# fukangl/SMG-multimodal-grasping

Hardware: AMD Instinct MI355X
Metric: affordance fwd+bwd passes/sec (16-rot 224^2 RGB-D) (higher is better)
Workload: dtype f32; 1 GPU; 16 rot x 224^2 (S=640): fwd + Huber + bwd + Adam per GPU per step; reinforcement_net style 0; 17 trunk passes; fp32; leg=headline, rotations=16, input_size=640, parallelism=dp1

## Files before the change

### smg-multimodal-grasping_amd/csrc/backward.hip

```cpp
#include "engine.h"

int do_backward(smg_engine* e, const smg_net* net, const float* dq, hipStream_t st, int phases, bool elem_head) {
    if (!e->have_fwd) return fail(-22, "smg_backward without a preceding smg_forward");
    if (!net->grads) return fail(-22, "net.grads is NULL");
    if (phases == 2 && !e->bw_phase0_done)
        return fail(-22, "smg_backward_phase(1) must follow smg_backward_phase(0) of the same forward");
    if ((phases & 1) && e->bw_phase0_done)
        return fail(-22, "smg_backward / smg_backward_phase(0) while the second half of a two-phase backward is still due (run phase 1 or a new forward)");
    const Layout& L = *e->L;
    const TrunkRef& T = L.trunk[e->f_trunk];
    const HeadRef& Hd = L.head[e->f_head];
    const int NS = e->f_streams, NP = e->f_pairs;
    const float* P = net->params;
    float* Gr = net->grads;
    const Plane p4 = e->p_blk[3];
    const bool ph_a = phases & 1, ph_b = phases & 2;
    if (ph_a) {
        for (int r = 0; r < kStatRep; ++r) HIP_OK(hipMemsetAsync(e->bstat + (size_t)r * kStatRepStride, 0, 2 * e->bstat_span * sizeof(double), st));
    }
    const bool split16 = e->prec == 0 && kSplitOp == 3;
    if (ph_a && split16) HIP_OK(hipMemsetAsync(e->gamax, 0, (size_t)e->gamax_words * sizeof(unsigned), st));
    const hipStream_t s2 = (e->prof || e->serialize) ? st : e->side;
    auto fork = [&](hipEvent_t ev) -> int {
        HIP_OK(hipEventRecord(ev, st));
// ... 96 lines not shown
        return LayerBuf{e->GS[r % kRing], e->D2[r % kRing], e->D2S[r % kRing], r};
    };
    auto fused_gsrc = [&](int b, const DenseLayerRef& d) {
        const int Ct = kBlockCtot[b];
        GradSrc g{};
        g.g = el(e, e->G[b], d.cin); g.ldg = Ct; g.x = el(e, e->X[b], d.cin); g.ldx = Ct;
        g.xsum = fsum(e, e->st_X[b]) + d.cin; g.xsq = fsq(e, e->st_X[b]) + d.cin;
        g.s1 = b1(e, e->st_X[b]) + d.cin; g.s2 = b2(e, e->st_X[b]) + d.cin; g.sstride = Ct; g.eps = kEps;
        return g;
    };
    auto issue_wgrads = [&](int b, int i) -> int {
        const Plane pl = e->p_blk[b];
        const int Ct = kBlockCtot[b];
        const DenseLayerRef& d = T.layers[b][i];
        float* bt = el(e, e->Bt, e->bt_off[b][i]);
        const LayerBuf lb = buf_of(b, i);
        const WgradPlan w = plan_layer_wgrads(pl, d.cin, NS, e->prec, split16, e->deterministic, e->part_floats, e->generic3x3, e->generic_w1);
        GradSrc gsrc{};
        if (gs_on_side(pl)) launch_gs_apply(b, i, s2, lb.GS);
        if (gs_materialised) { gsrc.g = lb.GS; gsrc.ldg = kGrowth; gsrc.amax = gamax_of(e, b, i, 0); }
        else gsrc = fused_gsrc(b, d);
        if (!e->generic3x3) {
            const PartialTiles::Slot at = tiles.place_halo3x3(w.w3.groups);
            if (at.refused) return fail(-12, tiles.refusal());
            launch_reduce2(e, s2, at.first);
            Halo3x3WgradArgs a;
            a.g = gsrc; a.pl = pl; a.src = bt; a.C = kBottleneck;
            a.bt = bn_table(e, e->sb_tab[b][i], e->max_streams, 0, kBottleneck, P + d.n2.w, P + d.n2.b);
            a.asc = asc_n2(e, b, i);
            a.tiles_x = w.w3.tiles_x; a.n_tiles = w.w3.n_tiles; a.tiles_per_wg = w.w3.tiles_per_wg;
            a.part = part_at(e, at);
            a.groups = w.w3.groups; a.streams = NS;
            const double flops = 2.0 * NS * pl.HW * 9 * kBottleneck * kGrowth, bytes = ESZ(e) * NS * pl.HW * (kGrowth + kBottleneck);
            if (w.w3.ts == 16) {
                PREC_DISPATCH(e, launch_kernel(e, conv3x3_halo_wgrad_kernel<16, PREC>, dim3(w.w3_grid), dim3(256), HaloWgradSGeo<16, PREC>::smem_bytes(), s2,
                                               K_W3, flops, bytes, false, a));
            } else {
                PREC_DISPATCH(e, launch_kernel(e, conv3x3_halo_wgrad_kernel<8, PREC>, dim3(w.w3_grid), dim3(256), HaloWgradSGeo<8, PREC>::smem_bytes(), s2,
                                               K_W3, flops, bytes, false, a));
            }
            launch_reduce2(e, s2, tiles.launched(at, reduce_tap_inner(a.part, w.w3.groups * NS, Gr + d.c2.w)));
        } else {
            int chunk, cps;
            pick_chunk(pl, NS, 9, chunk, cps);
            BwdWeightP<CfgW32x128, W_THREE, C_3x3, kPdWgrad, false> p{};
            p.gbuf = lb.GS; p.ldg = kGrowth; p.gcoff = 0; p.xbuf = nullptr; p.pa = pl; p.MA = kGrowth;
            p.bbuf = bt; p.ldb = kBottleneck; p.pb = pl; p.NB = kBottleneck;
            p.bsum = fsum(e, e->st_Bt[b][i]); p.bsq = fsq(e, e->st_Bt[b][i]); p.bstride = kBottleneck;
            p.bgamma = P + d.n2.w; p.bbeta = P + d.n2.b; p.eps = kEps;
            p.chunk = chunk; p.chunks_per_stream = cps; p.n_chunks = NS * cps;
            p.dw = Gr + d.c2.w; p.ldw_out = kBottleneck * 9;
            const dim3 grid(1, 1, 9 * NS * cps);
            if (int rc = launch_wgrad(e, s2, p, grid, K_W3, 2.0 * NS * pl.HW * 9 * kBottleneck * kGrowth,
                                      ESZ(e) * NS * pl.HW * (kGrowth + kBottleneck), 9, C_3x3, tiles, tiles.place_alone(wgrad_partial_floats(p, grid)))) return rc;
        }
        if (w.w1_ws) {
            using G = WswGeo;
            static_assert(G::BN == kW1WsTileN, "plan_layer_wgrads counts this kernel's column tiles");
            Wgrad1x1WsArgs a{};
            a.d2 = reinterpret_cast<const u32x4*>(lb.D2); a.binv = lb.D2S; a.x = e->X[b]; a.ldb = Ct; a.pl = pl; a.NB = d.cin;
            a.btab = stat_table(e, e->sx_tab[b], e->max_streams, Ct); a.bgamma = P + d.n1.w; a.bbeta = P + d.n1.b; a.basc = asc_n1(e, b, i);
            a.chunk = w.chunk; a.chunks_per_stream = w.cps; a.n_chunks = NS * w.cps;
            a.dw = Gr + d.c1.w; a.ldw_out = d.cin; a.ldp = w.nt * G::BN;
            const PartialTiles::Slot at = tiles.place_behind3x3((int64_t)a.n_chunks * G::BM * a.ldp);
            launch_reduce2(e, s2, at.first);
            if (at.refused) return fail(-12, tiles.refusal());
            a.part = part_at(e, at);
            a.tm = TileMap{a.n_chunks, w.nt, 0};
            launch_kernel(e, conv1x1_wgrad_ws_kernel, dim3(tile_grid(a.tm)), dim3(512), G::smem_bytes(w.chunk), s2, K_W1,
                          2.0 * NS * pl.HW * d.cin * kBottleneck, 4.0 * NS * pl.HW * (kBottleneck + d.cin), false, a);
            ReduceArgs red1{};
            if (a.part) red1 = reduce_chunk_major(a.part, a.n_chunks, 1, G::BM, d.cin, G::BM, a.ldp, a.dw, d.cin, C_IDENT);
            launch_reduce2(e, s2, tiles.launched(at, red1));
        } else {
            using Cfg = CfgW128x64;
            static_assert(Cfg::BN == kW1TileN, "plan_layer_wgrads counts this kernel's column tiles");
            auto go = [&](auto ptag) -> int {
                BwdWeightP<MC<Cfg, decltype(ptag)::value>, W_ONE, C_IDENT, kPdWgrad, false, decltype(ptag)::value> p{};
                p.gbuf = lb.D2; p.ldg = kBottleneck; p.gcoff = 0; p.xbuf = nullptr; p.pa = pl; p.MA = kBottleneck; p.binv = lb.D2S; p.basc = asc_n1(e, b, i);
                p.bbuf = e->X[b]; p.ldb = Ct; p.pb = pl; p.NB = d.cin;
                p.bsum = fsum(e, e->st_X[b]); p.bsq = fsq(e, e->st_X[b]); p.bstride = Ct; p.btab = stat_table(e, e->sx_tab[b], e->max_streams, Ct);
                p.bgamma = P + d.n1.w; p.bbeta = P + d.n1.b; p.eps = kEps;
                p.chunk = w.chunk; p.chunks_per_stream = w.cps; p.n_chunks = NS * w.cps;
                p.dw = Gr + d.c1.w; p.ldw_out = d.cin;
                const dim3 grid(1, w.nt, NS * w.cps);
                return launch_wgrad(e, s2, p, grid, K_W1, 2.0 * NS * pl.HW * d.cin * kBottleneck,
                                    ESZ(e) * NS * pl.HW * (kBottleneck + d.cin), 1, C_IDENT, tiles, tiles.place_behind3x3(wgrad_partial_floats(p, grid)));
            };
            PREC_DISPATCH(e, if (int rc = go(PTAG)) return rc);
        }
        return 0;
    };
    auto debug_stop = [&]() -> int {
        launch_reduce2(e, s2, tiles.drain());
        HIP_OK(hipEventRecord(e->ev_end, s2));
        HIP_OK(hipStreamWaitEvent(st, e->ev_end, 0));
        if (int rc = walk_status(e)) return rc;
        e->have_fwd = false; e->bw_phase0_done = false; e->prof_stage = -1;
        return 0;
    };
    const bool pooled_tail = e->prec == 0 && e->f_stem1 && !e->stem_plane_tail && (NS > 4 || e->deterministic);
    for (int b = ph_a ? 3 : 0; b >= (ph_b ? 0 : 1); --b) {
        e->prof_stage = b;
        const Plane pl = e->p_blk[b];
        const int Ct = kBlockCtot[b];
        if (e->dbg_stop == b * 100 + 50) return debug_stop();
        if (b == 0 && pooled_tail) {
            StemMomArgs a;
            a.img = e->img4; a.pi = e->p_img; a.ps = e->p_stem; a.part = e->mom_part;
            a.tiles_x = stem_mom_tiles_x(e->p_stem); a.n_tiles = stem_mom_tiles(e->p_stem); a.tiles_per_wg = kMomTilesPerWg;
            if (fork(e->ev_misc)) return -5;
            e->prof_stage = -1;
            launch_kernel(e, stem_moments_kernel, dim3(e->mom_groups, NS), dim3(256), 0, s2, K_OTHER, 0, 0, false, a);
            launch_kernel(e, stem_moments_sum_kernel, dim3((kMomOut + 255) / 256, NS), dim3(256), 0, s2, K_OTHER, 0, 0, false,
                          (const float*)e->mom_part, e->mom_groups, e->mom);
            e->prof_stage = b;
        }
        for (int i = (int)T.layers[b].size() - 1; i >= 0; --i) {
            const DenseLayerRef& d = T.layers[b][i];
            float* bt = el(e, e->Bt, e->bt_off[b][i]);
// ... 262 lines not shown
```

### smg-multimodal-grasping_amd/csrc/engine.h

```cpp
#pragma once
#include <hip/hip_runtime.h>

#include <algorithm>
#include <cmath>
#include <cstdio>
#include <cstdlib>
#include <cstring>
#include <string>
#include <type_traits>
#include <vector>

#include "../../include/smg_hip.h"
#include "elem.cuh"
#include "scene.cuh"
#include "gemm.cuh"
#include "halo.cuh"
#include "ws.cuh"
#include "wsw.cuh"
#include "plan.h"

using namespace smg;

int smg_fail(int code, const std::string& msg);
static inline int fail(int code, const std::string& msg) { return smg_fail(code, msg); }
// ... 23 lines not shown
using CfgW64x64 = GemmCfg<64, 64, 16, 2, 2, 1, false>;
using CfgW64x256 = GemmCfg<64, 256, 16, 2, 2, 1, false>;

template <class C, int PREC, int MUL = 2>
using MC = typename std::conditional<PREC == 0, C, GemmCfg<C::BM, C::BN, MUL * C::BK, C::WM, C::WN, C::WK, C::AT>>::type;
enum Kind {
    K_STEM = 0, K_C1, K_C3, K_TRANS, K_HEAD0, K_D3, K_W3, K_D1, K_W1, K_TW, K_TD, K_SW, K_HW0, K_HD0, K_OTHER, K_COUNT
};
static const char* kKindNames[K_COUNT] = {"stem7x7_fwd", "conv1x1_fwd", "conv3x3_fwd", "transition_fwd", "head_conv0_fwd",
                                          "conv3x3_dgrad", "conv3x3_wgrad", "conv1x1_dgrad", "conv1x1_wgrad",
                                          "transition_wgrad", "transition_dgrad", "stem_wgrad", "head_conv0_wgrad",
                                          "head_conv0_dgrad", "elementwise"};

constexpr int kGroup = GROUP_MAX;
constexpr int kRing = kGroup + 2;

constexpr int kDbRep = 8;
struct DbSeg { int64_t grad_off; int scr_off; int n; };

struct ProfRec { hipEvent_t a, b; int kind; double flops; int stage; double bytes; };

struct StatArr { int64_t off; int stride; };

struct smg_engine {
    int device = 0, S = 0, max_streams = 0, max_pairs = 0, head_out = 1;
    Plane p_img, p_stem, p_blk[4];
    int OH = 1, OW = 1;
    const Layout* L = nullptr;

    float* img4 = nullptr; float* stem = nullptr; float* X[4] = {}; float* Bt = nullptr;
    std::vector<int64_t> bt_off[4];
    unsigned char* argmax = nullptr;
    float* F = nullptr; float* H1 = nullptr;
    float* G[4] = {}; float* GS[kRing] = {}; float* D2[kRing] = {}; float* part = nullptr; int64_t part_floats = 0;
    float* DY2 = nullptr; float* D2S[kRing] = {};
    hipStream_t side = nullptr; hipEvent_t ev_gs[kRing] = {}, ev_d2[kRing] = {}, ev_side[kRing] = {}, ev_misc = nullptr, ev_end = nullptr; float* DY0 = nullptr; float* DH1 = nullptr; float* DF = nullptr;
    double* fstat = nullptr; int64_t fstat_span = 0;
    double* bstat = nullptr; int64_t bstat_span = 0;
    float* dbscr = nullptr; int db_total = 0; int db_off[4][24] = {}; int db_toff[3] = {}; struct DbSeg* d_dbseg = nullptr; int n_dbseg = 0;
    StatArr st_stem, st_X[4], st_F, st_H1; std::vector<StatArr> st_Bt[4];
    u32x4* packed_u = nullptr; int64_t packed_units = 0;
    float* packed_f = nullptr; int64_t packed_floats = 0;
    PackDesc* d_pack = nullptr; std::vector<PackDesc> h_pack[3]; std::vector<PackDesc> h_pack_head[3];
    int pack_stride = 0, bnupd_stride = 0, n_bnupd = 0;
    int64_t pk_conv0 = 0, pk_conv0_1 = 0, pk_head0 = 0, pk_hd0 = 0, pk_head1 = 0;
    std::vector<int64_t> pk_c1[4], pk_d1[4], pk_g3f[4], pk_g3d[4], pk_hf[4], pk_hd[4]; int64_t pk_t[3] = {}, pk_td[3] = {};
    int max_pack = 0;
    float* asc = nullptr; ActScaleDesc* d_asc = nullptr; int n_asc = 0;
    unsigned* gamax = nullptr; int64_t gamax_words = 0;
    float* stab = nullptr; int64_t stab_floats = 0;
    int64_t sx_tab[4] = {}, sb_tab[4][24] = {}, sf_tab = 0;
    BnUpdDesc* d_bnupd = nullptr;
    bool have_fwd = false; int f_trunk = 0, f_head = 0, f_streams = 0, f_pairs = 0;
    bool bw_phase0_done = false;
    bool f_dense_dq = false;
    int head_bwd = 0;
    bool f_stem1 = false;
    int* d_stream_image = nullptr; int* d_stream_rot = nullptr; int* d_pair_a = nullptr; int* d_pair_b = nullptr;
    int* d_seq_t = nullptr; int* d_seq_h = nullptr; int* d_user_ptr = nullptr; int* d_user_pair = nullptr; int* d_user_slot = nullptr;
    float* d_affine = nullptr;
    float* scene_val = nullptr; int* scene_idx = nullptr; int scene_tiles = 0;
    int* d_stage = nullptr; int* h_stage[2] = {}; hipEvent_t ev_stage[2] = {}; int stage_ints = 0, stage_turn = 0;
    int so_image = 0, so_rot = 0, so_pa = 0, so_pb = 0, so_seq_t = 0, so_seq_h = 0, so_uptr = 0, so_upair = 0, so_uslot = 0, so_aff = 0, so_ma = 0, so_mb = 0, so_adam = 0;
    bool capturing = false; int* h_stage_g = nullptr; hipEvent_t ev_graph = nullptr, ev_gin = nullptr; hipStream_t gstream = nullptr; struct StepGraph* step_graph = nullptr;
    int64_t workspace_bytes = 0;
    int n_cu = 256;
    int prec = 0;
// ... 123 lines not shown
    }
    TraceScope ts(st, kind, grid, traced, __PRETTY_FUNCTION__);
    ProfScope ps(e, st, kind, flops, bytes);
    hipLaunchKernelGGL(kernel, grid, block, smem, st, args...);
}

static int walk_status(smg_engine* e) {
    if (const int rc = e->launch_rc) { e->launch_rc = 0; return rc; }
    HIP_OK(hipGetLastError());
    return 0;
}

template <class P>
static void launch_gemm(smg_engine* e, hipStream_t st, P p, dim3 grid, int kind, double flops, double bytes) {
    const size_t smem = (size_t)(GeoOf<P>::TILE_FLOATS + p.param_floats()) * sizeof(float);
    p.tm = TileMap{0, 0, 0};
    if constexpr (P::kSwizzle == 1) {
        if (grid.y > 1 && grid.z == 1) {
            p.tm = TileMap{(int)grid.x, (int)grid.y, 0};
            grid = dim3(tile_grid(p.tm), 1, 1);
        }
    } else {
        p.gx = grid.x; p.gy = grid.y;
        const int tiles = grid.x * grid.y;
        if (tiles > 1) {
            p.tm = TileMap{(int)grid.z, tiles, (int)grid.x};
            grid = dim3(tile_grid(p.tm), 1, 1);
        }
    }
    launch_kernel(e, gemm_kernel<P>, dim3((unsigned)(grid.x * grid.y * grid.z)), dim3(256), smem, st, kind, flops, bytes, true, p, (int)grid.x, (int)grid.y);
}

static void launch_reduce2(smg_engine* e, hipStream_t st, const ReducePair& r) {
    const int ba = ReducePair::blocks(r.a), bb = ReducePair::blocks(r.b);
    if (ba + bb == 0) return;
    launch_kernel(e, reduce_partials_kernel, dim3(ba + bb), dim3(256), 0, st, K_OTHER, 0, 0, false, r.a, r.b, ba);
}

template <class P>
static int64_t wgrad_partial_floats(const P&, dim3 grid) {
    return (int64_t)grid.z * (grid.x * P::Cfg::BM) * ((int64_t)grid.y * P::Cfg::BN);
}
static inline float* part_at(const smg_engine* e, const PartialTiles::Slot& at) { return at.off >= 0 ? e->part + at.off : nullptr; }
template <class P>
static int launch_wgrad(smg_engine* e, hipStream_t st, P& p, dim3 grid, int kind, double flops, double bytes, int taps, int cmap,
                        PartialTiles& tiles, const PartialTiles::Slot& at) {
    using C = typename P::Cfg;
    launch_reduce2(e, st, at.first);
    if (at.refused)
        return fail(-12, tiles.refusal() + " (smaller batch per call, or a larger engine)");
    p.part = part_at(e, at);
    launch_gemm(e, st, p, grid, kind, flops, bytes);
    ReduceArgs r{};
    if (p.part) r = reduce_chunk_major(p.part, p.n_chunks, taps, p.MA, p.NB, (int64_t)grid.x * C::BM, (int64_t)grid.y * C::BN, p.dw, p.ldw_out, cmap);
    launch_reduce2(e, st, tiles.launched(at, r));
    return 0;
}

static inline float* el(const smg_engine* e, float* base, int64_t elems) {
    return reinterpret_cast<float*>(reinterpret_cast<char*>(base) + (e->prec ? 2 : 4) * elems);
}
static inline double* fsum(smg_engine* e, const StatArr& s) { return e->fstat + s.off; }
static inline double* fsq(smg_engine* e, const StatArr& s) { return e->fstat + e->fstat_span + s.off; }
static inline double* b1(smg_engine* e, const StatArr& s) { return e->bstat + s.off; }
static inline double* b2(smg_engine* e, const StatArr& s) { return e->bstat + e->bstat_span + s.off; }

static const float kEps = 1e-5f;

static inline int ring_pos(int b, int i) {
// ... 30 lines not shown
```

### smg-multimodal-grasping_amd/csrc/engine.hip

```cpp
#include "engine.h"

static thread_local std::string g_err;
int smg_fail(int code, const std::string& msg) { g_err = msg; return code; }

static int engine_build(smg_engine* e) {
    const Layout& L = *e->L;
    const int NS = e->max_streams, NP = e->max_pairs;
    const int S = e->S;
    const int H1 = (S - 1) / 2 + 1, H2 = (H1 - 1) / 2 + 1;
    e->p_img = make_plane(S, S);
    e->p_stem = make_plane(H1, H1);
    int h = H2;
    for (int b = 0; b < 4; ++b) { e->p_blk[b] = make_plane(h, h); h /= 2; }
    e->OH = e->OW = e->p_blk[3].H - kHeadKernel + 1;
    if (e->OH < 1) return fail(-22, "input_size too small for the 20x20 value head");

    if (getenv("SMG_SERIALIZE")) e->serialize = true;
    const int cross = getenv("SMG_CROSSCHECK") ? atoi(getenv("SMG_CROSSCHECK")) : 0;
    e->generic3x3 = cross & 1; e->generic_c1 = cross & 2; e->generic_w1 = cross & 4; e->stem_plane_tail = cross & 8;

    ALLOC(e->img4, (int64_t)NS * e->p_img.HWp * 4);
    ALLOC(e->stem, (int64_t)NS * e->p_stem.HWp * 64);
    ALLOC(e->DY0, (int64_t)NS * e->p_stem.HWp * 64);
    ALLOC(e->argmax, (int64_t)NS * e->p_blk[0].HWp * 64);
// ... 2 lines not shown
    ALLOC(e->mom_part, (int64_t)NS * e->mom_groups * kMomVals);
    ALLOC(e->mom, (int64_t)NS * kMomOut);
    int64_t bt_total = 0;
    for (int b = 0; b < 4; ++b) {
        ALLOC(e->X[b], (int64_t)NS * e->p_blk[b].HWp * kBlockCtot[b]);
        ALLOC(e->G[b], (int64_t)NS * e->p_blk[b].HWp * kBlockCtot[b]);
        for (int i = 0; i < kBlockLayers[b]; ++i) {
            e->bt_off[b].push_back(bt_total);
            bt_total += (int64_t)NS * e->p_blk[b].HWp * kBottleneck;
        }
    }
    ALLOC(e->Bt, bt_total);
    for (int k = 0; k < kRing; ++k) {
        ALLOC(e->D2[k], (int64_t)NS * e->p_blk[0].HWp * kBottleneck);
        ALLOC(e->GS[k], (int64_t)NS * e->p_blk[0].HWp * kGrowth);
        ALLOC(e->D2S[k], (int64_t)NS * (e->p_blk[0].HWp / kScaleBlock));
        HIP_OK(hipEventCreateWithFlags(&e->ev_gs[k], hipEventDisableTiming));
        HIP_OK(hipEventCreateWithFlags(&e->ev_d2[k], hipEventDisableTiming));
        HIP_OK(hipEventCreateWithFlags(&e->ev_side[k], hipEventDisableTiming));
    }
    ALLOC(e->DY2, (int64_t)NS * e->p_blk[0].HWp * kBottleneck);
    e->scene_tiles = (int)(((int64_t)(S / 2) * (S / 2) + kSceneTile - 1) / kSceneTile);
    ALLOC(e->scene_val, (int64_t)kSceneMaps * e->scene_tiles);
    ALLOC(e->scene_idx, (int64_t)kSceneMaps * e->scene_tiles);
    HIP_OK(hipEventCreateWithFlags(&e->ev_misc, hipEventDisableTiming));
    HIP_OK(hipEventCreateWithFlags(&e->ev_end, hipEventDisableTiming));
    HIP_OK(hipStreamCreateWithFlags(&e->side, hipStreamNonBlocking));
    e->part_floats = (int64_t)24 << 20;
    for (int b = 0; b < 4; ++b) {
        const Plane& pl = e->p_blk[b];
        for (int ts : {halo_tile(pl), 8})
            e->part_floats = std::max(e->part_floats, w3_partial_floats(w3_tiling(pl, ts, NS, INT64_MAX).groups, NS));
    }
    ALLOC(e->part, e->part_floats);
    ALLOC(e->F, (int64_t)NP * e->p_blk[3].HWp * 2 * kFeat);
    ALLOC(e->DF, (int64_t)NP * e->p_blk[3].HWp * 2 * kFeat);
    ALLOC(e->H1, (int64_t)NP * e->p_blk[3].HWp * kHeadMid);
    ALLOC(e->DH1, (int64_t)NP * e->p_blk[3].HWp * kHeadMid);

    int64_t off = 0;
    auto carve = [&](int n, int stride) { StatArr s{off, stride}; off += (int64_t)n * stride; return s; };
    e->st_stem = carve(NS, 64);
    for (int b = 0; b < 4; ++b) e->st_X[b] = carve(NS, kBlockCtot[b]);
    for (int b = 0; b < 4; ++b)
        for (int i = 0; i < kBlockLayers[b]; ++i) e->st_Bt[b].push_back(carve(NS, kBottleneck));
    e->st_F = carve(NP, 2 * kFeat);
    e->st_H1 = carve(NP, kHeadMid);
    e->fstat_span = e->bstat_span = off;
    if (2 * off > kStatRepStride) return fail(-22, "batch too large for the statistic arenas (kStatRepStride in gemm.cuh)");
    ALLOC(e->fstat, kFStatRep > 1 ? (int64_t)kFStatRep * kStatRepStride : 2 * off);
    ALLOC(e->bstat, (int64_t)kStatRep * kStatRepStride);
    {
        int at = 0;
        for (int b = 0; b < 4; ++b)
            for (int i = 0; i < kBlockLayers[b]; ++i) { e->db_off[b][i] = at; at += 2 * (kBlockCin[b] + i * kGrowth); }
        for (int b = 0; b < 3; ++b) { e->db_toff[b] = at; at += 2 * kBlockCtot[b]; }
        e->db_total = at;
        ALLOC(e->dbscr, (int64_t)kDbRep * at);
        HIP_OK(hipMemset(e->dbscr, 0, (size_t)kDbRep * at * sizeof(float)));
        e->n_dbseg = 2 * (6 + 12 + 24 + 16 + 3);
        HIP_OK(hipMalloc((void**)&e->d_dbseg, (size_t)3 * e->n_dbseg * sizeof(DbSeg)));
        for (int t = 0; t < 3; ++t) {
            const TrunkRef& T = L.trunk[t];
            if ((int)T.layers[0].size() != kBlockLayers[0]) continue;
            std::vector<DbSeg> v;
            for (int b = 0; b < 4; ++b)
// ... 586 lines not shown
        if (err != hipSuccess) rc = fail(-5, std::string("hipGraphLaunch: ") + hipGetErrorString(err));
        e->have_fwd = true; e->bw_phase0_done = false; e->f_trunk = trunk_id; e->f_head = head_id; e->f_streams = B->n_streams; e->f_pairs = B->n_pairs;
        e->f_stem1 = B->heightmaps_dev != nullptr; e->f_dense_dq = false;
    }
    e->capturing = false;
    if (rc == 0) {
        HIP_OK(hipEventRecord(e->ev_graph, st));
        HIP_OK(hipStreamWaitEvent(caller, e->ev_graph, 0));
    }
    return rc;
}

int smg_engine_set_precision(smg_engine* e, int precision) {
    if (!e) return fail(-22, "engine is NULL");
    if (precision < 0 || precision > 2) return fail(-22, "precision must be 0 (fp32 storage, fp32-class split products), 1 (bf16 storage) or 2 (fp16 activations, bf16 gradients)");
    if (precision && e->generic3x3) return fail(-22, "SMG_CROSSCHECK=1 (the generic implicit-GEMM 3x3 path) exists in the fp32-class mode only");
    e->prec = precision;
    step_graph_drop(e);
    e->have_fwd = false;
    e->bw_phase0_done = false;
    return 0;
}

int smg_engine_set_option(smg_engine* e, const char* name, int value) {
    if (!e || !name) return fail(-22, "NULL argument");
    const std::string s(name);
    if (s == "deterministic") { e->deterministic = value != 0; return 0; }
    if (s == "head_bwd") {
        if (value < 0 || value > 2) return fail(-22, "head_bwd must be 0 (follow the mark of smg_loss_map / smg_loss_map_ce), 1 (per-element form) or 2 (dense form)");
        e->head_bwd = value; return 0;
    }
    if (s == "serialize") { e->serialize = value != 0; return 0; }
    if (s == "debug_stop") { e->dbg_stop = value; return 0; }
    return fail(-22, "unknown engine option '" + s + "'");
}

int smg_heightmap(const double* depth_img_dev, int h, int w, const double* intrinsics3x3, const double* cam_pose4x4,
                  const double* inv_homography3x3, int out_w, int out_h, double* out_dev, void* stream) {
    if (!depth_img_dev || !intrinsics3x3 || !cam_pose4x4 || !inv_homography3x3 || !out_dev || h < 1 || w < 1 || out_w < 1 || out_h < 1)
        return fail(-22, "bad heightmap arguments");
    hipPointerAttribute_t attr;
    HIP_OK(hipPointerGetAttributes(&attr, depth_img_dev));
    HIP_OK(hipSetDevice(attr.device));
    HeightmapArgs a;
    a.depth = depth_img_dev; a.h = h; a.w = w;
    a.fx = intrinsics3x3[0]; a.fy = intrinsics3x3[4]; a.cx = intrinsics3x3[2]; a.cy = intrinsics3x3[5];
    a.r20 = cam_pose4x4[8]; a.r21 = cam_pose4x4[9]; a.r22 = cam_pose4x4[10]; a.t2 = cam_pose4x4[11];
    for (int i = 0; i < 9; ++i) a.mi[i] = inv_homography3x3[i];
    a.out = out_dev; a.ow = out_w; a.oh = out_h;
    hipLaunchKernelGGL(heightmap_warp_kernel, dim3((out_w + 255) / 256, out_h), dim3(256), 0, (hipStream_t)stream, a);
    HIP_OK(hipGetLastError());
    return 0;
}

int smg_argmax(const float* values_dev, int n, int* idx_out_dev, float* val_out_dev, void* stream) {
    if (!values_dev || !idx_out_dev || !val_out_dev || n < 1) return fail(-22, "bad argmax arguments");
    hipPointerAttribute_t attr;
    HIP_OK(hipPointerGetAttributes(&attr, values_dev));
    HIP_OK(hipSetDevice(attr.device));
    hipLaunchKernelGGL(argmax_kernel, dim3(1), dim3(256), 0, (hipStream_t)stream, values_dev, n, idx_out_dev, val_out_dev);
    HIP_OK(hipGetLastError());
    return 0;
}

int smg_adam_step(float* params, const float* grads, float* m, float* v, int64_t offset, int64_t count, int step, float lr,
                  float beta1, float beta2, float eps, void* stream) {
// ... 175 lines not shown
```

### smg-multimodal-grasping_amd/csrc/gemm.cuh

```cuda
#pragma once
#include <hip/hip_runtime.h>
#include <stdint.h>

#include <type_traits>

#include "wgrad_plan.h"

namespace smg {
constexpr int kDmaFlyDgrad = 2, kDmaFlyGroup = 1;
constexpr int kPdFwdSmall = 3;
constexpr int kPdFwdBig = 2;
constexpr int kPdDgrad = 2;
constexpr int kPdDgradBig = 2;
constexpr int kPdWgrad = 3;
constexpr int kPdDgradGroup = 1;
constexpr int kFwdBigMinWaves = 3;
}

namespace smg {

typedef float f32x16 __attribute__((ext_vector_type(16)));
typedef __bf16 bf16x8 __attribute__((ext_vector_type(8)));
typedef short s16x4 __attribute__((ext_vector_type(4)));
typedef unsigned u32x4 __attribute__((ext_vector_type(4)));
// ... 2216 lines not shown
        }
#pragma unroll
        for (int i = 0; i < Cfg::TM; ++i)
#pragma unroll
            for (int j = 0; j < Cfg::TN; ++j) {
                const int col = c.n0 + wn0 + j * 32 + l31;
#pragma unroll
                for (int r = 0; r < 16; ++r) {
                    const int row = c.m0 + SMG_ACC_ROW(wm0, i, r, half);
                    if (active && row < MA && col < NB) {
                        if (part) {
                            part[((int64_t)c.z * (gx * Cfg::BM) + row) * (gy * Cfg::BN) + col] = acc[i][j][r];
                            continue;
                        }
                        int64_t idx;
                        if constexpr (CMAP == C_IDENT) idx = (int64_t)row * ldw_out + col;
                        else if constexpr (CMAP == C_3x3) idx = (int64_t)row * ldw_out + col * 9 + c.tap;
                        else if constexpr (CMAP == C_STEM1) {
                            if (col >= 49) continue;
                            for (int cc = 0; cc < 3; ++cc) atomicAdd(dw + (int64_t)row * ldw_out + cc * 49 + col, acc[i][j][r]);
                            continue;
                        } else {
                            const int tap = col >> 2, cc = col & 3;
                            if (cc == 3 || tap >= 49) continue;
                            idx = (int64_t)row * ldw_out + cc * 49 + tap;
                        }
                        atomicAdd(dw + idx, acc[i][j][r]);
                    }
                }
            }
    }
};

static __global__ void reduce_partials_kernel(const ReduceArgs ra, const ReduceArgs rb, const int blocks_a) {
    __shared__ float red[3][64];
    const bool second = (int)blockIdx.x >= blocks_a;
    const ReduceArgs& a = second ? rb : ra;
    const int total = a.taps * a.rows * a.cols;
    const int lane = threadIdx.x & 63, w = threadIdx.x >> 6;
    {
        const int e0 = ((int)blockIdx.x - (second ? blocks_a : 0)) * 64;
        const int e = e0 + lane;
        const bool on = e < total;
        const int ec = on ? e : 0;
        const int tap = ec / (a.rows * a.cols);
        const int rc = ec - tap * a.rows * a.cols;
        const int row = rc / a.cols, col = rc - row * a.cols;
        const float* p = a.part + tap * a.tap_stride + (int64_t)row * a.ldp + col;
        float s0 = 0.f, s1 = 0.f, s2 = 0.f, s3 = 0.f;
        int z = w;
        for (; z + 12 < a.Z; z += 16) {
            s0 += p[(int64_t)z * a.z_stride];
            s1 += p[(int64_t)(z + 4) * a.z_stride];
            s2 += p[(int64_t)(z + 8) * a.z_stride];
            s3 += p[(int64_t)(z + 12) * a.z_stride];
        }
        for (; z < a.Z; z += 4) s0 += p[(int64_t)z * a.z_stride];
        float v = (s0 + s1) + (s2 + s3);
        if (w) red[w - 1][lane] = v;
        __syncthreads();
        if (w == 0 && on) {
            v = (v + red[0][lane]) + (red[1][lane] + red[2][lane]);
            int64_t idx = -1;
            if (a.cmap == C_IDENT) idx = (int64_t)row * a.ldw_out + col;
            else if (a.cmap == C_3x3) idx = (int64_t)row * a.ldw_out + col * 9 + tap;
            else if (a.cmap == C_STEM1) {
                if (col < 49)
                    for (int cc = 0; cc < 3; ++cc) a.dw[(int64_t)row * a.ldw_out + cc * 49 + col] += v;
            } else {
                const int t7 = col >> 2, cc = col & 3;
                if (cc != 3 && t7 < 49) idx = (int64_t)row * a.ldw_out + cc * 49 + t7;
            }
            if (idx >= 0) a.dw[idx] += v;
        }
        __syncthreads();
    }
}

}
```

### smg-multimodal-grasping_amd/csrc/halo.cuh

```cuda
#pragma once
#include "gemm.cuh"

namespace smg {

constexpr int kHaloFwdWaves = 2, kHaloWgradWaves = 2;

template <int TS>
struct HaloGeo {
    static_assert(TS == 16 || TS == 8, "tile side");
    static constexpr int T = TS, W = TS + 2, PX = W * W, NPIX = TS * TS;
    static constexpr int MT = NPIX == 256 ? 2 : 1;
    static constexpr int WQ = NPIX / (32 * MT);
    static constexpr int WX = 4 / WQ;
    static constexpr int ROWS = 32 / TS;
    static constexpr int RP = MT + 2;
    static constexpr int RSTEP = TS == 16 ? 2 : 0;
    __device__ static __forceinline__ int row(int wq, int m, int i) { return (wq * MT + m) * ROWS + i / TS; }
    __device__ static __forceinline__ int col(int i) { return i % TS; }
    __device__ static __forceinline__ int rowi(int wq, int m, int i) { return TS == 16 ? 4 * wq + m + 2 * (i / TS) : row(wq, m, i); }
    __device__ static __forceinline__ int pair0(int wq) { return 4 * wq; }
};

template <int B, int N, class F>
__device__ __forceinline__ void sfor(F&& f) {
// ... 783 lines not shown
    if constexpr (kDma) dma_wait<0>();
#ifdef SMG_TRACE_INIT
    if (trace) trace[6] = __builtin_amdgcn_s_memrealtime();
#else
    if (trace) { trace[4] = __builtin_amdgcn_s_memtime(); trace[6] = __builtin_amdgcn_s_memrealtime(); }
#endif
}


struct Halo3x3WgradArgs {
    GradSrc g; Plane pl;
    const void* src; int C;
    BnTab bt;
    const float* asc;
    float* part;
    int tiles_x, n_tiles, tiles_per_wg;
    int groups, streams;
};

template <int TW, int PREC> struct HaloWgradSGeo {
    static_assert(TW == 16 || TW == 8, "tile width");
    static constexpr int NP = np_of(bwd_op(PREC)), SPP = PREC ? 4 : 8;
    static constexpr int TH = 8, HW_ = TW + 2, HH = TH + 2, PX = HW_ * HH, NPIX = TW * TH;
    static constexpr int KSTEPS = NPIX / 16 / 4;
    static constexpr int B_BYTES = NP * PX * 64, A_BYTES = NP * NPIX * 64;
    static constexpr int B_N = (PX * SPP + 255) / 256, A_N = (NPIX * SPP + 255) / 256;
    static constexpr int RED_BYTES = 4 * 16 * 64 * 4;
    __host__ __device__ static constexpr int smem_bytes() {
        return (B_BYTES + A_BYTES > RED_BYTES ? B_BYTES + A_BYTES : RED_BYTES) + (96 + 128) * 4;
    }
};

template <int TW, int PREC = 0>
static __global__ __launch_bounds__(256, kHaloWgradWaves) void conv3x3_halo_wgrad_kernel(const Halo3x3WgradArgs a) {
    using G = HaloWgradSGeo<TW, PREC>;
    using GT = grd_t<PREC>;
    using XT = act_t<PREC>;
    constexpr int OP = bwd_op(PREC), NP = G::NP, SPP = G::SPP, E = 32 / SPP, GSZ = GT::size, XSZ = XT::size;
    constexpr int B_N = G::B_N, A_N = G::A_N;
    extern __shared__ __attribute__((aligned(16))) float smem[];
    char* Bh = reinterpret_cast<char*>(smem);
    char* Ag = Bh + G::B_BYTES;
    float* prm = reinterpret_cast<float*>(reinterpret_cast<char*>(smem) + G::smem_bytes()) - 96 - 128;
    float* gp = prm + 96;
    const int t = threadIdx.x, lane = t & 63, wave = t >> 6, half = lane >> 5;
    const int C = a.C;
    const int ncg = C / 32, xcd = blockIdx.x & 7, slot = blockIdx.x >> 3;
    const int gz = (slot / ncg) * 8 + xcd;
    if (gz >= a.groups * a.streams) return;
    const int n = gz / a.groups, bx = gz - n * a.groups, cc0 = (slot % ncg) * 32;
    u32x4 am4[kAmaxRep / 4];
    float sa = 1.f;
    if constexpr (OP == 3) {
#pragma unroll
        for (int r = 0; r < kAmaxRep / 4; ++r) am4[r] = *reinterpret_cast<const u32x4*>(a.g.amax + (int64_t)n * kAmaxRep + 4 * r);
        sa = a.asc[0];
    }
    auto grad_scale = [&]() -> ActScale {
        ActScale g{1.f, 1.f};
        if constexpr (OP == 3) {
            unsigned m = 0;
#pragma unroll
            for (int r = 0; r < kAmaxRep / 4; ++r) m = max(max(m, max(am4[r].x, am4[r].y)), max(am4[r].z, am4[r].w));
            g = scale_of_max(m);
            g.inv *= a.asc[1];
        }
        return g;
    };
    if (t < 32) {
        prm[t] = tab_mean(a.bt, n)[cc0 + t];
        prm[32 + t] = a.bt.gamma[cc0 + t] * tab_invstd(a.bt, n)[cc0 + t] * sa;
        prm[64 + t] = a.bt.beta[cc0 + t] * sa;
    }
    grad_src_params(a.g, n, a.pl.HW, gp);
    f32x16 acc[9];
#pragma unroll
    for (int k = 0; k < 9; ++k)
#pragma unroll
        for (int r = 0; r < 16; ++r) acc[k][r] = 0.f;
    const char* src_n = static_cast<const char*>(a.src) + (int64_t)XSZ * ((int64_t)n * a.pl.HWp * C + cc0);
// ... 141 lines not shown
```

### smg-multimodal-grasping_amd/csrc/wgrad_plan.h

```cpp
#pragma once
#include <cstdint>
#include <string>

#include "plan.h"

namespace smg {

struct Plane { int H, W, HW, HWp; };

enum { C_IDENT = 0, C_3x3 = 1, C_STEM = 2, C_STEM1 = 3 };

struct ReduceArgs {
    const float* part; int Z, taps, rows, cols, ldp; int64_t z_stride, tap_stride;
    float* dw; int ldw_out, cmap;
};
static inline ReduceArgs reduce_chunk_major(const float* part, int n_chunks, int taps, int rows, int cols, int64_t rows_padded, int64_t ldp,
                                            float* dw, int ldw_out, int cmap) {
    ReduceArgs r{};
    r.part = part; r.Z = n_chunks; r.taps = taps; r.rows = rows; r.cols = cols; r.ldp = (int)ldp;
    r.z_stride = rows_padded * ldp; r.tap_stride = (int64_t)n_chunks * rows_padded * ldp;
    r.dw = dw; r.ldw_out = ldw_out; r.cmap = cmap;
    return r;
}
static inline ReduceArgs reduce_tap_inner(const float* part, int n_tiles, float* dw) {
    ReduceArgs r{};
    r.part = part; r.Z = n_tiles; r.taps = 9; r.rows = kGrowth; r.cols = kBottleneck; r.ldp = kBottleneck;
    r.z_stride = (int64_t)9 * kGrowth * kBottleneck; r.tap_stride = (int64_t)kGrowth * kBottleneck;
    r.dw = dw; r.ldw_out = kBottleneck * 9; r.cmap = C_3x3;
    return r;
}
struct ReducePair {
    ReduceArgs a{}, b{};
    static int blocks(const ReduceArgs& r) { return r.Z ? (r.taps * r.rows * r.cols + 63) / 64 : 0; }
};

static inline void pick_chunk(const Plane& pl, int n_planes, int tiles_per_chunk, int& chunk, int& cps, int target = 768) {
    const int want = (target + tiles_per_chunk - 1) / tiles_per_chunk;
    cps = (want + n_planes - 1) / n_planes;
    if (cps < 1) cps = 1;
    chunk = ((pl.HW + cps - 1) / cps + 63) / 64 * 64;
    cps = (pl.HW + chunk - 1) / chunk;
}

static inline int halo_tile(const Plane& p, int n_streams = 1 << 20) {
    return (int64_t)((p.H + 15) / 16) * ((p.W + 15) / 16) * n_streams >= 200 ? 16 : 8;
}

static inline int64_t w3_partial_floats(int groups, int n_streams) { return (int64_t)groups * n_streams * 9 * 32 * kBottleneck; }

static inline int w3_tiles_per_wg(int n_tiles, int ts, int n_streams, int64_t part_floats, double fix_scale = 1.0) {
    const double fix = (ts == 16 ? 0.6 : 2.4) * fix_scale;
    double best = 1e30;
    int tpw_best = 1;
    for (int tpw = 1; tpw <= n_tiles; ++tpw) {
        const int g = (n_tiles + tpw - 1) / tpw;
        const int rounds = (g * (kBottleneck / 32) * n_streams + 511) / 512;
        const double cost = rounds * (tpw + fix);
        if (cost < best - 1e-9) { best = cost; tpw_best = tpw; }
    }
    while (tpw_best < n_tiles && w3_partial_floats((n_tiles + tpw_best - 1) / tpw_best, n_streams) > part_floats) ++tpw_best;
    return tpw_best;
}

constexpr int kW3TileH = 8;
struct W3Tiling { int ts, tiles_x, n_tiles, tiles_per_wg, groups; };
static inline W3Tiling w3_tiling(const Plane& pl, int ts, int n_streams, int64_t part_floats) {
// ... 1 lines not shown
    t.ts = ts;
    t.tiles_x = (pl.W + ts - 1) / ts; t.n_tiles = ((pl.H + kW3TileH - 1) / kW3TileH) * t.tiles_x;
    t.tiles_per_wg = w3_tiles_per_wg(t.n_tiles, ts, n_streams, part_floats, (double)ts / kW3TileH);
    t.groups = (t.n_tiles + t.tiles_per_wg - 1) / t.tiles_per_wg;
    return t;
}

constexpr int kW1WsTileN = 128, kW1TileN = 64;

struct WgradPlan {
    W3Tiling w3; unsigned w3_grid;
    bool w1_ws; int nt, chunk, cps;
};
static inline WgradPlan plan_layer_wgrads(const Plane& pl, int cin, int NS, int prec, bool split16, bool deterministic, int64_t part_floats,
                                          bool generic3x3, bool generic_w1) {
    WgradPlan w{};
    if (!generic3x3) {
        w.w3 = w3_tiling(pl, halo_tile(pl, NS), NS, part_floats);
        w.w3_grid = (unsigned)(((w.w3.groups * NS + 7) / 8) * 8 * (kBottleneck / 32));
    }
    w.w1_ws = split16 && !generic_w1 && cin > 64 && (deterministic || NS > 4);
    if (w.w1_ws) {
        w.nt = (cin + kW1WsTileN - 1) / kW1WsTileN;
        pick_chunk(pl, NS, w.nt, w.chunk, w.cps, 320);
    } else {
        w.nt = (cin + kW1TileN - 1) / kW1TileN;
        pick_chunk(pl, NS, w.nt, w.chunk, w.cps, (prec && NS >= 16) ? 160 : (NS <= 4 && !deterministic) ? 128 : 320);
    }
    return w;
}

class PartialTiles {
public:
    enum Kind { ALONE, HALO3, HALO3_PAIRED, BEHIND3 };
    struct Slot {
        Kind kind; int64_t off;
        int64_t size;
        ReducePair first;
        bool refused;
    };
    PartialTiles(int64_t floats_, int n_streams, bool deterministic_) : floats(floats_), NS(n_streams), deterministic(deterministic_) {}

    Slot place_alone(int64_t need) {
        Slot s{ALONE, need <= floats ? 0 : -1, need, drain(), false};
        if (s.off < 0 && deterministic) s.refused = refuse(need, floats);
        return s;
    }
    Slot place_halo3x3(int groups) {
        Slot s{HALO3, 0, w3_partial_floats(groups, NS), ReducePair{}, false};
        if (s.size > floats) { s.refused = refuse(-1, floats); return s; }
        if (!deterministic && NS <= 4 && s.size * 2 <= floats) s.kind = HALO3_PAIRED;
        if (s.kind == HALO3) s.first = drain();
        else if (half) s.off = floats / 2;
        return s;
    }
    Slot place_behind3x3(int64_t need) {
        Slot s{BEHIND3, cursor, need, ReducePair{}, false};
        const bool partial = deterministic || NS > 4;
        if (held.Z && (!partial || s.off + need > floats)) { s.first.a = held; held.Z = 0; s.off = 0; }
        const int64_t have = floats - s.off;
        if (!partial || need > have) s.off = -1;
        if (partial && s.off < 0 && deterministic) s.refused = refuse(need, have);
        return s;
    }
    ReducePair launched(const Slot& s, const ReduceArgs& r) {
        ReducePair due;
        if (s.kind == ALONE) due.a = r;
        else if (s.kind == BEHIND3) { due.a = held; due.b = r; held.Z = 0; cursor = 0; }
        else if (s.kind == HALO3) { held = r; cursor = s.size; }
        else {
            if (carried.Z) { due.a = carried; due.b = r; carried.Z = 0; }
            else carried = r;
            half ^= 1;
        }
        return due;
    }
    ReducePair drain() { ReducePair due; due.a = carried; carried.Z = 0; return due; }
    std::string refusal() const {
        if (refusal_need < 0) return "partial-gradient workspace too small";
        return "deterministic: a weight-gradient launch needs " + std::to_string(refusal_need) + " partial-tile floats, the workspace holds " +
               std::to_string(refusal_have);
    }

private:
    bool refuse(int64_t need, int64_t have) { refusal_need = need; refusal_have = have; return true; }
    int64_t floats; int NS; bool deterministic;
    ReduceArgs carried{};
    ReduceArgs held{};
    int64_t cursor = 0;
    int half = 0;
    int64_t refusal_need = 0, refusal_have = 0;
};

}
```

### smg-multimodal-grasping_amd/csrc/wsw.cuh

```cuda
#pragma once
#include "gemm.cuh"

namespace smg {

struct Wgrad1x1WsArgs {
    const u32x4* d2; const float* binv;
    const float* x; int ldb; Plane pl; int NB;
    StatTab btab; const float* bgamma; const float* bbeta; const float* basc;
    int chunk, chunks_per_stream, n_chunks;
    float* dw; int ldw_out;
    float* part; int ldp;
    TileMap tm;
};

struct WswGeo {
    static constexpr int BM = 128, BN = 128, BK = 32;
    static constexpr int PLANE = BK + 4;
    static constexpr int LDTB = BN + 32;
    static constexpr int A_BYTES = 2 * (BM / 8) * PLANE * 16, B_BYTES = 2 * BK * LDTB * 2;
    static constexpr int A_N = 2 * (BM / 8) * BK / 256, B_N = BK * (BN / 4) / 256;
    static constexpr int TILE_BYTES = 2 * (A_BYTES + B_BYTES);
    __host__ __device__ static constexpr int smem_bytes(int chunk) { return TILE_BYTES + (3 * BN + chunk / kScaleBlock + 1) * 4; }
};

static __global__ __launch_bounds__(512, 1) void conv1x1_wgrad_ws_kernel(const Wgrad1x1WsArgs a) {
    using G = WswGeo;
    extern __shared__ __attribute__((aligned(16))) float smem[];
    char* As = reinterpret_cast<char*>(smem);
    char* Bs = As + 2 * G::A_BYTES;
    float* bp = reinterpret_cast<float*>(As + G::TILE_BYTES);
    float* sinv = bp + 3 * G::BN;
    const int t = threadIdx.x, role = t >> 8, tp = t & 255, lane = t & 63, wave = (t >> 6) & 3, half = lane >> 5;
    int z, nt;
    tile_decode(a.tm, blockIdx.x, z, nt);
    const int n = sgpr(z / a.chunks_per_stream);
    const int p0 = sgpr((z - n * a.chunks_per_stream) * a.chunk);
    if (p0 >= a.pl.HW) return;
    const int n0 = sgpr(nt * G::BN);
    int len = a.pl.HWp - p0;
    len = len < a.chunk ? len : a.chunk;
    const int KT = sgpr(len / G::BK);

    const u32x4* d2n = a.d2 + d2_stream_units(n, a.pl.HWp);
    const float* xn = a.x + (int64_t)n * a.pl.HWp * a.ldb;
    const unsigned d2_bytes = 16u * (unsigned)(2 * kD2K8 * a.pl.HWp), x_bytes = 4u * (unsigned)(a.pl.HW * a.ldb);
    unsigned a_voff[G::A_N], b_voff[G::B_N];
#pragma unroll
    for (int i = 0; i < G::A_N; ++i) {
        const int id = tp + 256 * i, kr = id % G::BK, q = id / G::BK;
        a_voff[i] = 16u * (unsigned)(q * a.pl.HWp + kr);
    }
    const int bq = tp % (G::BN / 4), bl = tp / (G::BN / 4);
#pragma unroll
    for (int i = 0; i < G::B_N; ++i) b_voff[i] = 4u * (unsigned)((bl + 8 * i) * a.ldb + n0 + 4 * bq);
    u32x4 ra[2][G::A_N]; float4 rb[2][G::B_N];
    auto g_load = [&](int kt, u32x4 (&xa)[G::A_N], float4 (&xb)[G::B_N]) {
#pragma unroll
        for (int i = 0; i < G::A_N; ++i) xa[i] = bload_u4(d2n, d2_bytes, a_voff[i], 16u * (unsigned)(p0 + kt * G::BK));
#pragma unroll
        for (int i = 0; i < G::B_N; ++i) xb[i] = bload4(xn, x_bytes, b_voff[i], 4u * (unsigned)((p0 + kt * G::BK) * a.ldb));
    };
    KPrm3 bfix{};
    auto s_store = [&](int buf, const u32x4 (&xa)[G::A_N], const float4 (&xb)[G::B_N]) {
        char* A = As + buf * G::A_BYTES;
        char* B = Bs + buf * G::B_BYTES;
#pragma unroll
        for (int i = 0; i < G::A_N; ++i) {
// ... 141 lines not shown
```

Baseline: 64.64 passes/s.

## Fold pending partial reductions into wgrad kernel launches as rider blocks

```diff
diff --git a/smg-multimodal-grasping_amd/csrc/backward.hip b/smg-multimodal-grasping_amd/csrc/backward.hip
--- a/smg-multimodal-grasping_amd/csrc/backward.hip
+++ b/smg-multimodal-grasping_amd/csrc/backward.hip
@@ -152,12 +152,13 @@
             a.part = part_at(e, at);
             a.groups = w.w3.groups; a.streams = NS;
             const double flops = 2.0 * NS * pl.HW * 9 * kBottleneck * kGrowth, bytes = ESZ(e) * NS * pl.HW * (kGrowth + kBottleneck);
+            const int n_ride = at.riders.blocks();
             if (w.w3.ts == 16) {
-                PREC_DISPATCH(e, launch_kernel(e, conv3x3_halo_wgrad_kernel<16, PREC>, dim3(w.w3_grid), dim3(256), HaloWgradSGeo<16, PREC>::smem_bytes(), s2,
-                                               K_W3, flops, bytes, false, a));
+                PREC_DISPATCH(e, launch_kernel(e, conv3x3_halo_wgrad_kernel<16, PREC>, dim3(n_ride + w.w3_grid), dim3(256), HaloWgradSGeo<16, PREC>::smem_bytes(), s2,
+                                               K_W3, flops, bytes, false, a, at.riders, n_ride));
             } else {
-                PREC_DISPATCH(e, launch_kernel(e, conv3x3_halo_wgrad_kernel<8, PREC>, dim3(w.w3_grid), dim3(256), HaloWgradSGeo<8, PREC>::smem_bytes(), s2,
-                                               K_W3, flops, bytes, false, a));
+                PREC_DISPATCH(e, launch_kernel(e, conv3x3_halo_wgrad_kernel<8, PREC>, dim3(n_ride + w.w3_grid), dim3(256), HaloWgradSGeo<8, PREC>::smem_bytes(), s2,
+                                               K_W3, flops, bytes, false, a, at.riders, n_ride));
             }
             launch_reduce2(e, s2, tiles.launched(at, reduce_tap_inner(a.part, w.w3.groups * NS, Gr + d.c2.w)));
         } else {
@@ -182,13 +183,14 @@
             a.btab = stat_table(e, e->sx_tab[b], e->max_streams, Ct); a.bgamma = P + d.n1.w; a.bbeta = P + d.n1.b; a.basc = asc_n1(e, b, i);
             a.chunk = w.chunk; a.chunks_per_stream = w.cps; a.n_chunks = NS * w.cps;
             a.dw = Gr + d.c1.w; a.ldw_out = d.cin; a.ldp = w.nt * G::BN;
-            const PartialTiles::Slot at = tiles.place_behind3x3((int64_t)a.n_chunks * G::BM * a.ldp);
+            const PartialTiles::Slot at = tiles.place_behind3x3((int64_t)a.n_chunks * G::BM * a.ldp, true);
             launch_reduce2(e, s2, at.first);
             if (at.refused) return fail(-12, tiles.refusal());
             a.part = part_at(e, at);
             a.tm = TileMap{a.n_chunks, w.nt, 0};
-            launch_kernel(e, conv1x1_wgrad_ws_kernel, dim3(tile_grid(a.tm)), dim3(512), G::smem_bytes(w.chunk), s2, K_W1,
-                          2.0 * NS * pl.HW * d.cin * kBottleneck, 4.0 * NS * pl.HW * (kBottleneck + d.cin), false, a);
+            const int n_ride = (at.riders.blocks() + kWswRideBlocks - 1) / kWswRideBlocks;
+            launch_kernel(e, conv1x1_wgrad_ws_kernel, dim3(n_ride + tile_grid(a.tm)), dim3(512), G::smem_bytes(w.chunk), s2, K_W1,
+                          2.0 * NS * pl.HW * d.cin * kBottleneck, 4.0 * NS * pl.HW * (kBottleneck + d.cin), false, a, at.riders, n_ride);
             ReduceArgs red1{};
             if (a.part) red1 = reduce_chunk_major(a.part, a.n_chunks, 1, G::BM, d.cin, G::BM, a.ldp, a.dw, d.cin, C_IDENT);
             launch_reduce2(e, s2, tiles.launched(at, red1));
@@ -205,7 +207,7 @@
                 p.dw = Gr + d.c1.w; p.ldw_out = d.cin;
                 const dim3 grid(1, w.nt, NS * w.cps);
                 return launch_wgrad(e, s2, p, grid, K_W1, 2.0 * NS * pl.HW * d.cin * kBottleneck,
-                                    ESZ(e) * NS * pl.HW * (kBottleneck + d.cin), 1, C_IDENT, tiles, tiles.place_behind3x3(wgrad_partial_floats(p, grid)));
+                                    ESZ(e) * NS * pl.HW * (kBottleneck + d.cin), 1, C_IDENT, tiles, tiles.place_behind3x3(wgrad_partial_floats(p, grid), false));
             };
             PREC_DISPATCH(e, if (int rc = go(PTAG)) return rc);
         }
diff --git a/smg-multimodal-grasping_amd/csrc/engine.h b/smg-multimodal-grasping_amd/csrc/engine.h
--- a/smg-multimodal-grasping_amd/csrc/engine.h
+++ b/smg-multimodal-grasping_amd/csrc/engine.h
@@ -79,7 +79,7 @@
     std::vector<int64_t> bt_off[4];
     unsigned char* argmax = nullptr;
     float* F = nullptr; float* H1 = nullptr;
-    float* G[4] = {}; float* GS[kRing] = {}; float* D2[kRing] = {}; float* part = nullptr; int64_t part_floats = 0;
+    float* G[4] = {}; float* GS[kRing] = {}; float* D2[kRing] = {}; float* part = nullptr; int64_t part_floats = 0, part_alloc = 0;
     float* DY2 = nullptr; float* D2S[kRing] = {};
     hipStream_t side = nullptr; hipEvent_t ev_gs[kRing] = {}, ev_d2[kRing] = {}, ev_side[kRing] = {}, ev_misc = nullptr, ev_end = nullptr; float* DY0 = nullptr; float* DH1 = nullptr; float* DF = nullptr;
     double* fstat = nullptr; int64_t fstat_span = 0;
@@ -269,9 +269,9 @@
 }
 
 static void launch_reduce2(smg_engine* e, hipStream_t st, const ReducePair& r) {
-    const int ba = ReducePair::blocks(r.a), bb = ReducePair::blocks(r.b);
-    if (ba + bb == 0) return;
-    launch_kernel(e, reduce_partials_kernel, dim3(ba + bb), dim3(256), 0, st, K_OTHER, 0, 0, false, r.a, r.b, ba);
+    const int nb = r.blocks();
+    if (nb == 0) return;
+    launch_kernel(e, reduce_partials_kernel, dim3(nb), dim3(256), 0, st, K_OTHER, 0, 0, false, r);
 }
 
 template <class P>
diff --git a/smg-multimodal-grasping_amd/csrc/engine.hip b/smg-multimodal-grasping_amd/csrc/engine.hip
--- a/smg-multimodal-grasping_amd/csrc/engine.hip
+++ b/smg-multimodal-grasping_amd/csrc/engine.hip
@@ -58,6 +58,7 @@
         for (int ts : {halo_tile(pl), 8})
             e->part_floats = std::max(e->part_floats, w3_partial_floats(w3_tiling(pl, ts, NS, INT64_MAX).groups, NS));
     }
+    e->part_alloc = e->part_floats;
     ALLOC(e->part, e->part_floats);
     ALLOC(e->F, (int64_t)NP * e->p_blk[3].HWp * 2 * kFeat);
     ALLOC(e->DF, (int64_t)NP * e->p_blk[3].HWp * 2 * kFeat);
@@ -710,6 +711,10 @@
     }
     if (s == "serialize") { e->serialize = value != 0; return 0; }
     if (s == "debug_stop") { e->dbg_stop = value; return 0; }
+    if (s == "debug_part_floats") {
+        if (value < 0 || value > e->part_alloc) return fail(-22, "debug_part_floats must lie in [0, the allocated partial-tile floats]");
+        e->part_floats = value ? value : e->part_alloc; return 0;
+    }
     return fail(-22, "unknown engine option '" + s + "'");
 }
 
diff --git a/smg-multimodal-grasping_amd/csrc/gemm.cuh b/smg-multimodal-grasping_amd/csrc/gemm.cuh
--- a/smg-multimodal-grasping_amd/csrc/gemm.cuh
+++ b/smg-multimodal-grasping_amd/csrc/gemm.cuh
@@ -2272,30 +2272,31 @@
     }
 };
 
-static __global__ void reduce_partials_kernel(const ReduceArgs ra, const ReduceArgs rb, const int blocks_a) {
-    __shared__ float red[3][64];
-    const bool second = (int)blockIdx.x >= blocks_a;
-    const ReduceArgs& a = second ? rb : ra;
-    const int total = a.taps * a.rows * a.cols;
-    const int lane = threadIdx.x & 63, w = threadIdx.x >> 6;
+__device__ __forceinline__ void reduce_partials_block(const ReducePair& r, const int blk, float (*red)[64], const int lane, const int w) {
+    const int blocks_a = ReducePair::blocks(r.a);
+    const bool second = blk >= blocks_a;
+    const ReduceArgs& a = second ? r.b : r.a;
+    const int total = a.Z ? a.taps * a.rows * a.cols : 0;
     {
-        const int e0 = ((int)blockIdx.x - (second ? blocks_a : 0)) * 64;
+        const int e0 = (blk - (second ? blocks_a : 0)) * 64;
         const int e = e0 + lane;
         const bool on = e < total;
         const int ec = on ? e : 0;
-        const int tap = ec / (a.rows * a.cols);
-        const int rc = ec - tap * a.rows * a.cols;
-        const int row = rc / a.cols, col = rc - row * a.cols;
+        const int rcn = total ? a.rows * a.cols : 1, cn = total ? a.cols : 1;
+        const int tap = ec / rcn;
+        const int rc = ec - tap * rcn;
+        const int row = rc / cn, col = rc - row * cn;
         const float* p = a.part + tap * a.tap_stride + (int64_t)row * a.ldp + col;
         float s0 = 0.f, s1 = 0.f, s2 = 0.f, s3 = 0.f;
         int z = w;
-        for (; z + 12 < a.Z; z += 16) {
+        const int Z = total ? a.Z : 0;
+        for (; z + 12 < Z; z += 16) {
             s0 += p[(int64_t)z * a.z_stride];
             s1 += p[(int64_t)(z + 4) * a.z_stride];
             s2 += p[(int64_t)(z + 8) * a.z_stride];
             s3 += p[(int64_t)(z + 12) * a.z_stride];
         }
-        for (; z < a.Z; z += 4) s0 += p[(int64_t)z * a.z_stride];
+        for (; z < Z; z += 4) s0 += p[(int64_t)z * a.z_stride];
         float v = (s0 + s1) + (s2 + s3);
         if (w) red[w - 1][lane] = v;
         __syncthreads();
@@ -2313,8 +2314,12 @@
             }
             if (idx >= 0) a.dw[idx] += v;
         }
-        __syncthreads();
-    }
-}
-
-}
+    }
+}
+
+static __global__ void reduce_partials_kernel(const ReducePair r) {
+    __shared__ float red[3][64];
+    reduce_partials_block(r, (int)blockIdx.x, red, threadIdx.x & 63, threadIdx.x >> 6);
+}
+
+}
diff --git a/smg-multimodal-grasping_amd/csrc/halo.cuh b/smg-multimodal-grasping_amd/csrc/halo.cuh
--- a/smg-multimodal-grasping_amd/csrc/halo.cuh
+++ b/smg-multimodal-grasping_amd/csrc/halo.cuh
@@ -839,7 +839,7 @@
 };
 
 template <int TW, int PREC = 0>
-static __global__ __launch_bounds__(256, kHaloWgradWaves) void conv3x3_halo_wgrad_kernel(const Halo3x3WgradArgs a) {
+static __global__ __launch_bounds__(256, kHaloWgradWaves) void conv3x3_halo_wgrad_kernel(const Halo3x3WgradArgs a, const ReducePair ride, const int n_ride) {
     using G = HaloWgradSGeo<TW, PREC>;
     using GT = grd_t<PREC>;
     using XT = act_t<PREC>;
@@ -851,8 +851,13 @@
     float* prm = reinterpret_cast<float*>(reinterpret_cast<char*>(smem) + G::smem_bytes()) - 96 - 128;
     float* gp = prm + 96;
     const int t = threadIdx.x, lane = t & 63, wave = t >> 6, half = lane >> 5;
+    const int wg = (int)blockIdx.x - n_ride;
+    if (wg < 0) {
+        reduce_partials_block(ride, (int)blockIdx.x, reinterpret_cast<float (*)[64]>(smem), lane, wave);
+        return;
+    }
     const int C = a.C;
-    const int ncg = C / 32, xcd = blockIdx.x & 7, slot = blockIdx.x >> 3;
+    const int ncg = C / 32, xcd = wg & 7, slot = wg >> 3;
     const int gz = (slot / ncg) * 8 + xcd;
     if (gz >= a.groups * a.streams) return;
     const int n = gz / a.groups, bx = gz - n * a.groups, cc0 = (slot % ncg) * 32;
diff --git a/smg-multimodal-grasping_amd/csrc/wgrad_plan.h b/smg-multimodal-grasping_amd/csrc/wgrad_plan.h
--- a/smg-multimodal-grasping_amd/csrc/wgrad_plan.h
+++ b/smg-multimodal-grasping_amd/csrc/wgrad_plan.h
@@ -3,6 +3,12 @@
 #include <string>
 
 #include "plan.h"
+
+#ifdef __HIPCC__
+#define SMG_HD __host__ __device__
+#else
+#define SMG_HD
+#endif
 
 namespace smg {
 
@@ -31,7 +37,8 @@
 }
 struct ReducePair {
     ReduceArgs a{}, b{};
-    static int blocks(const ReduceArgs& r) { return r.Z ? (r.taps * r.rows * r.cols + 63) / 64 : 0; }
+    SMG_HD static int blocks(const ReduceArgs& r) { return r.Z ? (r.taps * r.rows * r.cols + 63) / 64 : 0; }
+    SMG_HD int blocks() const { return blocks(a) + blocks(b); }
 };
 
 static inline void pick_chunk(const Plane& pl, int n_planes, int tiles_per_chunk, int& chunk, int& cps, int target = 768) {
@@ -99,50 +106,52 @@
 
 class PartialTiles {
 public:
-    enum Kind { ALONE, HALO3, HALO3_PAIRED, BEHIND3 };
+    enum Kind { ALONE, HALO3, BEHIND3 };
     struct Slot {
         Kind kind; int64_t off;
         int64_t size;
         ReducePair first;
         bool refused;
+        ReducePair riders;
     };
     PartialTiles(int64_t floats_, int n_streams, bool deterministic_) : floats(floats_), NS(n_streams), deterministic(deterministic_) {}
 
     Slot place_alone(int64_t need) {
-        Slot s{ALONE, need <= floats ? 0 : -1, need, drain(), false};
+        Slot s{ALONE, need <= floats ? 0 : -1, need, drain(), false, ReducePair{}};
         if (s.off < 0 && deterministic) s.refused = refuse(need, floats);
         return s;
     }
     Slot place_halo3x3(int groups) {
-        Slot s{HALO3, 0, w3_partial_floats(groups, NS), ReducePair{}, false};
+        Slot s{HALO3, 0, w3_partial_floats(groups, NS), ReducePair{}, false, ReducePair{}};
         if (s.size > floats) { s.refused = refuse(-1, floats); return s; }
-        if (!deterministic && NS <= 4 && s.size * 2 <= floats) s.kind = HALO3_PAIRED;
-        if (s.kind == HALO3) s.first = drain();
-        else if (half) s.off = floats / 2;
+        if (half && s.size * 2 <= floats) s.off = floats / 2;
+        hand_over(s, true);
         return s;
     }
-    Slot place_behind3x3(int64_t need) {
-        Slot s{BEHIND3, cursor, need, ReducePair{}, false};
+    Slot place_behind3x3(int64_t need, bool carries) {
+        Slot s{BEHIND3, cursor, need, ReducePair{}, false, ReducePair{}};
         const bool partial = deterministic || NS > 4;
-        if (held.Z && (!partial || s.off + need > floats)) { s.first.a = held; held.Z = 0; s.off = 0; }
+        if (s.off + need > floats) s.off = 0;
         const int64_t have = floats - s.off;
         if (!partial || need > have) s.off = -1;
+        hand_over(s, carries);
         if (partial && s.off < 0 && deterministic) s.refused = refuse(need, have);
         return s;
     }
     ReducePair launched(const Slot& s, const ReduceArgs& r) {
         ReducePair due;
-        if (s.kind == ALONE) due.a = r;
-        else if (s.kind == BEHIND3) { due.a = held; due.b = r; held.Z = 0; cursor = 0; }
-        else if (s.kind == HALO3) { held = r; cursor = s.size; }
-        else {
-            if (carried.Z) { due.a = carried; due.b = r; carried.Z = 0; }
-            else carried = r;
-            half ^= 1;
+        if (s.kind == ALONE) { due.a = r; cursor = 0; return due; }
+        if (r.Z) {
+            if (pending.a.Z && pending.b.Z) due = drain();
+            const bool second = pending.a.Z != 0;
+            (second ? pending.b : pending.a) = r;
+            (second ? range_b : range_a) = Range{s.off, s.size};
         }
+        if (s.kind == HALO3) { cursor = s.off + s.size; half ^= 1; }
+        else cursor = 0;
         return due;
     }
-    ReducePair drain() { ReducePair due; due.a = carried; carried.Z = 0; return due; }
+    ReducePair drain() { ReducePair due = pending; pending = ReducePair{}; return due; }
     std::string refusal() const {
         if (refusal_need < 0) return "partial-gradient workspace too small";
         return "deterministic: a weight-gradient launch needs " + std::to_string(refusal_need) + " partial-tile floats, the workspace holds " +
@@ -150,10 +159,16 @@
     }
 
 private:
+    struct Range { int64_t off, size; };
+    static bool overlap(const ReduceArgs& r, const Range& g, const Slot& s) { return r.Z && s.off < g.off + g.size && g.off < s.off + s.size; }
+    void hand_over(Slot& s, bool carries) {
+        if (s.off >= 0 && (overlap(pending.a, range_a, s) || overlap(pending.b, range_b, s))) s.first = drain();
+        else if (carries) s.riders = drain();
+    }
     bool refuse(int64_t need, int64_t have) { refusal_need = need; refusal_have = have; return true; }
     int64_t floats; int NS; bool deterministic;
-    ReduceArgs carried{};
-    ReduceArgs held{};
+    ReducePair pending{};
+    Range range_a{}, range_b{};
     int64_t cursor = 0;
     int half = 0;
     int64_t refusal_need = 0, refusal_have = 0;
diff --git a/smg-multimodal-grasping_amd/csrc/wsw.cuh b/smg-multimodal-grasping_amd/csrc/wsw.cuh
--- a/smg-multimodal-grasping_amd/csrc/wsw.cuh
+++ b/smg-multimodal-grasping_amd/csrc/wsw.cuh
@@ -23,7 +23,9 @@
     __host__ __device__ static constexpr int smem_bytes(int chunk) { return TILE_BYTES + (3 * BN + chunk / kScaleBlock + 1) * 4; }
 };
 
-static __global__ __launch_bounds__(512, 1) void conv1x1_wgrad_ws_kernel(const Wgrad1x1WsArgs a) {
+constexpr int kWswRideBlocks = 2;
+
+static __global__ __launch_bounds__(512, 1) void conv1x1_wgrad_ws_kernel(const Wgrad1x1WsArgs a, const ReducePair ride, const int n_ride) {
     using G = WswGeo;
     extern __shared__ __attribute__((aligned(16))) float smem[];
     char* As = reinterpret_cast<char*>(smem);
@@ -31,8 +33,13 @@
     float* bp = reinterpret_cast<float*>(As + G::TILE_BYTES);
     float* sinv = bp + 3 * G::BN;
     const int t = threadIdx.x, role = t >> 8, tp = t & 255, lane = t & 63, wave = (t >> 6) & 3, half = lane >> 5;
+    const int wg = (int)blockIdx.x - n_ride;
+    if (wg < 0) {
+        reduce_partials_block(ride, kWswRideBlocks * (int)blockIdx.x + role, reinterpret_cast<float (*)[64]>(smem) + 3 * role, lane, wave);
+        return;
+    }
     int z, nt;
-    tile_decode(a.tm, blockIdx.x, z, nt);
+    tile_decode(a.tm, wg, z, nt);
     const int n = sgpr(z / a.chunks_per_stream);
     const int p0 = sgpr((z - n * a.chunks_per_stream) * a.chunk);
     if (p0 >= a.pl.HW) return;
```

After: 63.61 passes/s. -1.6%, worse.
